# ooowedyn/InkLayer

Hardware: AMD Instinct MI355X
Metric: sketches/sec end-to-end (GroundingDINO+SAM) at 1024x1024 (higher is better)
Workload: dtype f16 (MFMA, f32 accumulate; f32 residual/norm/softmax; split-f16 = fp32-grade operands for patch-embed, neck, mask decoder); 1 GPU; full GroundingDINO Swin-T + SAM ViT-H pipeline, batch=8 per GPU, 1024x1024 synthetic sketches, 16 boxes/sketch, random-init weights; global_batch=8, parallelism=image-parallel x1

## Files before the change

### include/inklayer_hip.h

```cpp
#ifndef INKLAYER_HIP_H
#define INKLAYER_HIP_H

#include <stdint.h>

#ifdef __cplusplus
extern "C" {
#endif

#define INK_ABI_VERSION 8
int ink_abi_version(void);

typedef struct InkGemm {
  const void* A;
  const void* W;
  const float* bias;
  const float* col_scale;
  const float* residual;
  const int32_t* row_map;
  void* C;
  int32_t M, N, K;
  int32_t lda, ldw, ldr, ldc;
  int32_t act;
  int32_t c_f16;
} InkGemm;
// ... 119 lines not shown
                     int64_t ldo, void* stream);

int ink_attn_fewq(const void* Q, int64_t ldq, const void* K, int64_t ldk, const void* V, int64_t ldv,
                  int32_t n_batch, int32_t n_q, int32_t n_k, int32_t n_heads, int32_t head_dim, float scale,
                  const int32_t* q_batch_rows, const int32_t* kv_batch_rows, const float* k_add, void* O, int64_t ldo,
                  void* stream);

int ink_biattn_colstats(const float* scores, int32_t B, int32_t S, int32_t HT, float* part_ws, float* stats, void* stream);

int ink_fusion_fold_workspace(int32_t B, int32_t S, int64_t* out_floats);
int ink_fusion_fold(float* v_f32, int32_t B, int32_t S, const float* lnv_g, const float* lnv_b, float eps,
                    const float* text_k_f32, const float* text_vl_f32, int64_t ld_text, int32_t T, const void* Wq_f16,
                    const float* bq, const void* Wvv_f16, const float* bvv, const void* Wo_f16, const float* bo,
                    const float* gamma_v, float scale, float* ws, void* out_l_f16, const float* pos, void* out16_pos,
                    void* out16, void* stream);

int ink_sam_upscale_pack(const void* ws_f16, void* blob_f16, void* stream);
int ink_sam_upscale_tail(const float* u0, int64_t ld_tok, int32_t n, int32_t g, const float* ln_g, const float* ln_b, float eps,
                         const void* blob_f16, const float* b3, const float* hyper, int32_t n_masks, float* low,
                         void* stream);

int ink_proj256_ln_pack(const void* ws_f16, void* blob_f16, void* stream);
int ink_proj256_ln(const float* a_f32, const void* blob_f16, const float* bias, const float* res_f32,
                   const int32_t* res_batch_rows, int32_t rows_per_batch, const float* ln_g, const float* ln_b, float eps,
                   int64_t rows, float* out_f32, void* out_split_f16, void* stream);

int ink_ffn256_pack_bytes(int32_t hid, int32_t with_pre, int64_t* out_bytes);
int ink_ffn256_pack(const void* w1_f16, const float* b1, const void* w2_f16, int32_t hid, const void* wpre_f16, void* blob,
                    void* stream);
int ink_ffn256_fused(const void* x_f16, int64_t ldx, const float* res_f32, const void* blob, const float* b2,
                     const float* ln_g, const float* ln_b, float eps, int32_t M, int32_t hid, const float* pre_bias,
                     const float* pre_ln_g, const float* pre_ln_b, float* out_f32, void* stream);

int ink_topk_rowmax(const float* logits, int32_t B, int32_t S, int32_t T, int32_t K, int32_t* out_idx,
                    float* out_val, void* cand_ws, void* stream);

int ink_sine_embed4(const float* ref, const float* dim_t, int32_t N, void* out_f16, void* stream);

int ink_box_refine(const float* delta, int64_t ldd, const float* ref, int32_t N, int32_t ref_is_logit,
                   float* out, void* stream);

int ink_mask_cleanup_workspace_ints(int32_t n, int32_t H, int32_t W, int32_t k, int64_t* out_ints);
int ink_mask_cleanup(const void* masks_u8, int32_t n, int32_t H, int32_t W, int32_t k, int32_t area_threshold,
                     double aspect_threshold, void* tmp_a_u8, void* tmp_b_u8, int32_t* workspace, void* out_u8,
                     void* stream);

int ink_mask_sketch_iou_counts(const void* masks_u8, const void* sketch_rgb_u8, int32_t n, int32_t H, int32_t W,
                               void* bits_ws_u64, int32_t* counts, void* stream);

int ink_sam_amg_stats(const float* low, int32_t n, const int32_t* index, int32_t m, const int32_t* m_dev, int32_t S,
                      int32_t L, int32_t in_h, int32_t in_w, int32_t crop_h, int32_t crop_w, double thr, double offset,
                      int32_t x0, int32_t y0, int32_t orig_h, int32_t orig_w, int32_t* table, void* planes_u64,
                      float* out_logits, void* stream);

int ink_mask_rle_counts(const void* planes_u64, const int32_t* select, int32_t k, int32_t H, int32_t W,
                        int32_t* n_counts, void* stream);
int ink_mask_rle_write(const void* planes_u64, const int32_t* select, int32_t k, int32_t H, int32_t W,
                       const int32_t* offsets, int32_t* counts, void* stream);

int ink_mask_small_regions_workspace_ints(int32_t k, int32_t H, int32_t W, int64_t* out_ints);
int ink_mask_small_regions(const void* planes_u64, int32_t k, int32_t H, int32_t W, int32_t min_area, int32_t holes,
                           void* tmp_planes_u64, int32_t* workspace, void* out_planes_u64, int32_t* changed, void* stream);

int ink_box_nms(const float* boxes, const float* scores, int32_t n, float iou_threshold, void* workspace_u64,
                int32_t* keep, int32_t* n_keep, void* stream);

// ... 114 lines not shown
```

### inklayer_amd/_lib.py

```python
from __future__ import annotations

import ctypes as C
import os
from pathlib import Path

_LIB_PATH = Path(__file__).resolve().parent / "lib" / "libinklayer_hip.so"
_lib = None

c_void_p, c_int, c_i64, c_float = C.c_void_p, C.c_int32, C.c_int64, C.c_float


class InkGemm(C.Structure):
    _fields_ = [
        ("A", c_void_p), ("W", c_void_p), ("bias", c_void_p), ("col_scale", c_void_p),
        ("residual", c_void_p), ("row_map", c_void_p), ("C", c_void_p),
        ("M", c_int), ("N", c_int), ("K", c_int),
        ("lda", c_int), ("ldw", c_int), ("ldr", c_int), ("ldc", c_int),
        ("act", c_int), ("c_f16", c_int),
    ]


class InkAttn(C.Structure):
    _fields_ = [
        ("Q", c_void_p), ("K", c_void_p), ("V", c_void_p), ("O", c_void_p),
# ... 40 lines not shown
                               c_void_p],
    "ink_box_nms": [c_void_p, c_void_p, c_int, c_float, c_void_p, c_void_p, c_void_p, c_void_p],
    "ink_ms_deform_attn_forward": [c_void_p, C.POINTER(c_i64), C.POINTER(c_i64), c_void_p, c_void_p, c_int,
                                   c_int, c_int, c_int, c_int, c_int, c_int, c_int, c_void_p, c_void_p],
    "ink_ms_deform_attn_forward_dev": [c_void_p, c_void_p, c_void_p, c_void_p, c_void_p, c_int, c_int, c_int, c_int,
                                       c_int, c_int, c_int, c_int, c_int, c_void_p, c_void_p],
    "ink_ms_deform_attn_backward_dev": [c_void_p, c_void_p, c_void_p, c_void_p, c_void_p, c_void_p, c_int, c_int, c_int,
                                        c_int, c_int, c_int, c_int, c_int, c_int, c_void_p, c_void_p, c_void_p,
                                        c_void_p],
    "ink_msda_fused": [c_void_p, c_void_p, c_i64, c_void_p, c_int, c_i64, c_i64, C.POINTER(c_int), c_int,
                       c_int, c_int, c_void_p, c_void_p],
    "ink_swin_patchify": [c_void_p, c_int, c_int, C.POINTER(c_float), C.POINTER(c_float), c_void_p, c_void_p],
    "ink_layernorm_merge4": [c_void_p, c_i64, c_void_p, c_void_p, c_float, c_void_p, c_int, c_int, c_void_p,
                             c_void_p],
    "ink_groupnorm_nhwc": [c_void_p, c_int, c_int, c_int, c_int, c_void_p, c_void_p, c_float, c_void_p,
                           c_void_p, c_i64, c_void_p],
    "ink_gather_rows": [c_void_p, c_i64, c_i64, c_void_p, c_i64, c_int, c_int, c_int, c_void_p, c_void_p,
                        c_void_p],
    "ink_biattn_fusion": [c_void_p, c_void_p, c_int, c_int, c_int, c_int, c_float, c_void_p, c_void_p,
                          c_void_p, c_int, c_void_p, c_void_p, c_void_p],
    "ink_biattn_colstats": [c_void_p, c_int, c_int, c_int, c_void_p, c_void_p, c_void_p],
    "ink_fusion_fold_workspace": [c_int, c_int, C.POINTER(c_i64)],
    "ink_relpos_bias64_f16": [c_void_p, c_i64, c_void_p, c_void_p, c_int, c_int, c_int, c_float, c_void_p, c_void_p, c_void_p],
    "ink_proj256_ln_pack": [c_void_p, c_void_p, c_void_p],
    "ink_proj256_ln": [c_void_p, c_void_p, c_void_p, c_void_p, c_void_p, c_int, c_void_p, c_void_p, c_float, c_i64, c_void_p,
                       c_void_p, c_void_p],
    "ink_sam_upscale_pack": [c_void_p, c_void_p, c_void_p],
    "ink_sam_upscale_tail": [c_void_p, c_i64, c_int, c_int, c_void_p, c_void_p, c_float, c_void_p, c_void_p, c_void_p,
                             c_int, c_void_p, c_void_p],
    "ink_ffn256_pack_bytes": [c_int, c_int, C.POINTER(c_i64)],
    "ink_ffn256_pack": [c_void_p, c_void_p, c_void_p, c_int, c_void_p, c_void_p, c_void_p],
    "ink_ffn256_fused": [c_void_p, c_i64, c_void_p, c_void_p, c_void_p, c_void_p, c_void_p, c_float, c_int, c_int,
                         c_void_p, c_void_p, c_void_p, c_void_p, c_void_p],
    "ink_fusion_fold": [c_void_p, c_int, c_int, c_void_p, c_void_p, c_float, c_void_p, c_void_p, c_i64, c_int, c_void_p,
                        c_void_p, c_void_p, c_void_p, c_void_p, c_void_p, c_void_p, c_float, c_void_p, c_void_p, c_void_p,
                        c_void_p, c_void_p, c_void_p],
    "ink_attn_fewkeys": [c_void_p, c_i64, c_void_p, c_i64, c_void_p, c_i64, c_int, c_int, c_int, c_int, c_int,
                         c_float, c_void_p, c_void_p, c_void_p, c_int, c_void_p, c_i64, c_void_p],
    "ink_attn_fewq": [c_void_p, c_i64, c_void_p, c_i64, c_void_p, c_i64, c_int, c_int, c_int, c_int, c_int,
                      c_float, c_void_p, c_void_p, c_void_p, c_void_p, c_i64, c_void_p],
    "ink_topk_rowmax": [c_void_p, c_int, c_int, c_int, c_int, c_void_p, c_void_p, c_void_p, c_void_p],
    "ink_sine_embed4": [c_void_p, c_void_p, c_int, c_void_p, c_void_p],
    "ink_box_refine": [c_void_p, c_i64, c_void_p, c_int, c_int, c_void_p, c_void_p],
    "ink_mask_cleanup_workspace_ints": [c_int, c_int, c_int, c_int, C.POINTER(c_i64)],
    "ink_mask_cleanup": [c_void_p, c_int, c_int, c_int, c_int, c_int, C.c_double, c_void_p, c_void_p, c_void_p,
                         c_void_p, c_void_p],
    "ink_mask_sketch_iou_counts": [c_void_p, c_void_p, c_int, c_int, c_int, c_void_p, c_void_p, c_void_p],
    "ink_refine_sketch_planes": [c_void_p, c_int, c_int, c_void_p, c_void_p, c_void_p],
    "ink_bitplane_pack": [c_void_p, c_int, c_int, c_int, c_int, c_void_p, c_void_p],
    "ink_refine_depth_samples": [c_void_p, c_int, c_void_p, c_void_p, c_int, c_int, c_int, c_void_p, c_void_p, c_void_p],
    "ink_refine_pair_tables": [c_void_p, c_void_p, c_int, c_int, c_int, c_void_p, c_void_p, c_void_p, c_void_p,
                               c_void_p, c_void_p],
    "ink_refine_composite": [c_void_p, c_void_p, c_int, c_int, c_int, c_void_p, c_void_p, c_void_p],
    "ink_refine_relabel_clean": [c_void_p, c_void_p, c_int, c_int, c_void_p, c_void_p],
    "ink_refine_grow_workspace": [c_int, c_int, C.POINTER(c_i64), C.POINTER(c_i64)],
    "ink_refine_grow": [c_void_p, c_void_p, c_int, c_int, c_void_p, c_void_p, c_void_p, c_void_p, c_void_p, c_void_p,
                        c_int, c_void_p, c_void_p],
    "ink_refine_query_dists": [c_void_p, c_void_p, c_void_p, c_int, c_int, c_int, c_void_p, c_void_p],
    "ink_refine_finalize": [c_void_p, c_void_p, c_int, c_void_p, c_int, c_int, c_void_p, c_void_p, c_void_p, c_void_p],
    "ink_host_sparse_sample": [c_void_p, c_int, c_int, c_void_p, c_int, c_void_p],
    "ink_host_assign_unlabeled": [c_void_p, c_int, c_void_p, c_int, c_void_p, c_void_p, c_void_p, c_int, c_void_p],
    "ink_depth_patchify": [c_void_p, c_int, c_int, c_int, c_int, c_int, c_int, C.POINTER(C.c_double), C.POINTER(C.c_double),
                           c_int, c_void_p, c_void_p],
    "ink_resize_bilinear_ac_nhwc": [c_void_p, c_int, c_int, c_int, c_int, c_int, c_int, c_void_p, c_void_p, c_void_p],
    "ink_im2col3x3_ex_f16": [c_void_p, c_int, c_int, c_int, c_int, c_int, c_int, c_void_p, c_void_p],
    "ink_layers_otsu_planes": [c_void_p, c_int, c_int, c_int, c_int, c_void_p, c_void_p, c_void_p, c_void_p],
# ... 64 lines not shown
```

### inklayer_amd/build.py

```python
from __future__ import annotations

import os
import subprocess
import sys
from concurrent.futures import ThreadPoolExecutor
from pathlib import Path

ROOT = Path(__file__).resolve().parent
CSRC = ROOT / "csrc"
LIBDIR = ROOT / "lib"
OBJDIR = LIBDIR / "obj"
LIB = LIBDIR / "libinklayer_hip.so"
HIPCC = os.environ.get("HIPCC", "/opt/rocm/bin/hipcc")
FLAGS = ["--offload-arch=gfx950", "-O3", "-std=c++17", "-fPIC", "-ffp-contract=off",
         "-mllvm", "-amdgpu-mfma-vgpr-form",

         "-Wall", "-Wno-unused-function", "-Wno-unused-variable"]


def _newest_header() -> float:
    hs = list(CSRC.glob("*.h")) + list((ROOT.parent / "include").glob("*.h"))
    return max(h.stat().st_mtime for h in hs)


NO_SPILL = {"ffn_fused.hip", "proj_ln.hip", "amg.hip", "layers.hip", "inpaint_ops.hip", "visualize.hip"}


def _check_no_spill(src: Path, remarks: str) -> None:
    name = None
    for line in remarks.splitlines():
        if "Function Name:" in line:
            name = line.split("Function Name:")[1].split("[")[0].strip()
        elif "ScratchSize [bytes/lane]:" in line:
            n = int(line.split("ScratchSize [bytes/lane]:")[1].split("[")[0])
            if n != 0:
                raise RuntimeError(f"{src.name}: kernel {name} spills ({n} bytes of scratch per lane) - the kernels of "
                                   f"this file must stay in registers (see NO_SPILL); reduce register pressure")


def _compile(src: Path, force: bool, hdr_time: float) -> Path:
    obj = OBJDIR / (src.stem + ".o")
    if (not force and obj.exists() and obj.stat().st_mtime > src.stat().st_mtime
            and obj.stat().st_mtime > hdr_time):
        return obj
    guard = src.name in NO_SPILL
    cmd = [HIPCC, *FLAGS, *(["-Rpass-analysis=kernel-resource-usage", "-fno-caret-diagnostics"] if guard else []), "-c", str(src), "-o", str(obj)]
    r = subprocess.run(cmd, capture_output=True, text=True)
    if r.returncode != 0:
        raise RuntimeError(f"hipcc failed for {src.name}:\n{r.stdout}\n{r.stderr}")
    err = r.stderr
    if guard:
        try:
            _check_no_spill(src, err)
        except RuntimeError:
            obj.unlink(missing_ok=True)
            raise
        err = "\n".join(l for l in err.splitlines()
                        if "kernel-resource-usage" not in l and not l.startswith("In file included from"))
# ... 28 lines not shown
```

### inklayer_amd/gdino.py

```python
from __future__ import annotations

import math
from dataclasses import dataclass
from typing import Dict, List, Optional, Sequence, Tuple

import numpy as np
import torch

from . import ops
from ._lru import LRU

F16, F32, I32 = torch.float16, torch.float32, torch.int32


@dataclass
class GDinoConfig:
    embed_dim: int = 96
    depths: Tuple[int, ...] = (2, 2, 6, 2)
    num_heads: Tuple[int, ...] = (3, 6, 12, 24)
    window_size: int = 7
    out_indices: Tuple[int, ...] = (1, 2, 3)
    hidden_dim: int = 256
    nheads: int = 8
    enc_layers: int = 6
# ... 137 lines not shown
            refs.append(torch.stack((rx.reshape(-1) / ww, ry.reshape(-1) / hh), -1))
            gy, gx = torch.meshgrid(torch.linspace(0, hh - 1, hh), torch.linspace(0, ww - 1, ww), indexing="ij")
            grid = (torch.stack((gx, gy), -1) + 0.5) / torch.tensor([float(ww), float(hh)])
            props.append(torch.cat((grid, torch.ones_like(grid) * 0.05 * (2.0 ** lvl)), -1).view(-1, 4))
        self.enc_ref = torch.cat(refs, 0).to(dev).contiguous()
        pr = torch.cat(props, 0)
        valid = ((pr > 0.01) & (pr < 0.99)).all(-1)
        pr = torch.log(pr / (1 - pr)).masked_fill(~valid[:, None], float("inf"))
        self.props_unsig = pr.to(dev).contiguous()
        self.valid_map = torch.where(valid, torch.arange(self.S), torch.full((self.S,), -1)).to(I32).to(dev)


def swin_dense_bias(table: torch.Tensor, ws: int, nh: int, scale: float) -> torch.Tensor:
    co = torch.stack(torch.meshgrid(torch.arange(ws), torch.arange(ws), indexing="ij")).flatten(1)
    rel = (co[:, :, None] - co[:, None, :]).permute(1, 2, 0).contiguous()
    rel[:, :, 0] += ws - 1
    rel[:, :, 1] += ws - 1
    rel[:, :, 0] *= 2 * ws - 1
    rel_index = rel.sum(-1).view(-1)
    bias = torch.zeros((nh, ws * ws, 64))
    bias[:, :, :ws * ws] = table[rel_index].view(ws * ws, ws * ws, nh).permute(2, 0, 1) / scale
    return bias


def clean_state_dict(sd: Dict[str, torch.Tensor]) -> Dict[str, torch.Tensor]:
    if any(k.startswith("module.") for k in sd):
        return {(k[7:] if k.startswith("module.") else k): v for k, v in sd.items()}
    return sd


class GDinoEngine:
    fuse_ffn = True
    fuse_ffn_pre = True
    fold_fusion = True

    def __init__(self, state_dict: Dict[str, torch.Tensor], cfg: Optional[GDinoConfig] = None,
                 device: str | torch.device = "cuda", encoded_text: Optional[torch.Tensor] = None,
                 token_ids: Sequence[int] = DEFAULT_TOKEN_IDS):
        cfg = cfg or GDinoConfig()
        self.cfg, self.dev = cfg, torch.device(device)
        assert self.dev.type == "cuda", "the InkLayer detector runs on MI355X only"
        assert cfg.hidden_dim == 256 and cfg.nheads == 8 and cfg.num_feature_levels == 4 and cfg.n_points == 4
        assert all(cfg.embed_dim * 2 ** i // nh == 32 for i, nh in enumerate(cfg.num_heads))
        sd, dev = clean_state_dict(state_dict), self.dev
        self.w: Dict[str, torch.Tensor] = {}
        w = self.w

        def h(name, shape=None):
            t = sd[name].detach().to(torch.float32)
            return (t.reshape(shape) if shape is not None else t).to(dev, F16).contiguous()

        def f(name):
            return ops.own_f32(sd[name], dev)

        def lin(dst, src):
            w[dst + ".w"], w[dst + ".b"] = h(src + ".weight"), f(src + ".bias")

        def ln(dst, src):
            w[dst + ".w"], w[dst + ".b"] = f(src + ".weight"), f(src + ".bias")

        def cat_lin(dst, srcs):
            w[dst + ".w"] = torch.cat([h(s + ".weight") for s in srcs]).contiguous()
            w[dst + ".b"] = torch.cat([f(s + ".bias") for s in srcs]).contiguous()

        bb = "backbone.0."
        pw = sd[bb + "patch_embed.proj.weight"].detach().to(torch.float32).cpu().reshape(cfg.embed_dim, 48)
        w["pe.w"] = torch.cat([pw, torch.zeros(cfg.embed_dim, 16)], 1).to(dev, F16).contiguous()
        w["pe.b"] = f(bb + "patch_embed.proj.bias")
        ln("pe.norm", bb + "patch_embed.norm")
        ws = cfg.window_size
        scale = 32 ** -0.5
        for i, (dep, nh) in enumerate(zip(cfg.depths, cfg.num_heads)):
            for b in range(dep):
                p, d = f"{bb}layers.{i}.blocks.{b}.", f"s{i}b{b}"
                ln(d + ".norm1", p + "norm1")
                ln(d + ".norm2", p + "norm2")
                lin(d + ".qkv", p + "attn.qkv")
                lin(d + ".proj", p + "attn.proj")
                lin(d + ".fc1", p + "mlp.fc1")
                lin(d + ".fc2", p + "mlp.fc2")
                tab = sd[p + "attn.relative_position_bias_table"].detach().to(torch.float32).cpu()
                w[d + ".bias"] = swin_dense_bias(tab, ws, nh, scale).to(dev).contiguous()
            if i < len(cfg.depths) - 1:
                ln(f"s{i}.merge.norm", f"{bb}layers.{i}.downsample.norm")
                w[f"s{i}.merge.w"] = h(f"{bb}layers.{i}.downsample.reduction.weight")
            if i in cfg.out_indices:
                ln(f"s{i}.outnorm", f"{bb}norm{i}")
        for l in range(cfg.num_feature_levels):
            cw = sd[f"input_proj.{l}.0.weight"].detach().to(torch.float32)
            if cw.shape[-1] == 1:
                w[f"ip{l}.w"] = cw.reshape(cw.shape[0], cw.shape[1]).to(dev, F16).contiguous()
            else:
                w[f"ip{l}.w"] = cw.permute(0, 2, 3, 1).reshape(cw.shape[0], -1).to(dev, F16).contiguous()
            w[f"ip{l}.b"] = f(f"input_proj.{l}.0.bias")
            ln(f"ip{l}.gn", f"input_proj.{l}.1")
        t = "transformer."
        self.level_embed_cpu = sd[t + "level_embed"].detach().to(torch.float32).cpu()

        def msda(dst, src):
            cat_lin(dst + ".proj", [src + "sampling_offsets", src + "attention_weights"])
            lin(dst + ".value", src + "value_proj")
            lin(dst + ".out", src + "output_proj")

        def mha(dst, src):
            W, b = sd[src + "in_proj_weight"].detach().to(torch.float32), sd[src + "in_proj_bias"].detach().to(torch.float32)
            D = W.shape[1]
            w[dst + ".qk.w"], w[dst + ".qk.b"] = W[:2 * D].to(dev, F16).contiguous(), b[:2 * D].to(dev).contiguous()
            w[dst + ".q.w"], w[dst + ".q.b"] = W[:D].to(dev, F16).contiguous(), b[:D].to(dev).contiguous()
            w[dst + ".kv.w"], w[dst + ".kv.b"] = W[D:].to(dev, F16).contiguous(), b[D:].to(dev).contiguous()
            w[dst + ".v.w"], w[dst + ".v.b"] = W[2 * D:].to(dev, F16).contiguous(), b[2 * D:].to(dev).contiguous()
            lin(dst + ".out", src + "out_proj")

        for i in range(cfg.enc_layers):
            p, d = f"{t}encoder.layers.{i}.", f"e{i}"
            msda(d + ".msda", p + "self_attn.")
# ... 75 lines not shown
            torch.cuda.current_stream(self.dev).wait_stream(side)
            graph = torch.cuda.CUDAGraph()
            with torch.cuda.graph(graph):
                out = self._forward_eager(static_in)
            g = (graph, static_in, out, self.plan(h, w_, B))
            self._graphs.put(key, g)
        graph, static_in, out = g[:3]
        for dst, src in zip(static_in, images_u8):
            dst.copy_(src)
        graph.replay()
        return out[0].clone(), out[1].clone()

    def plan(self, h: int, w: int, B: int) -> _Plan:
        return self._plans.get_or_make((h, w, B), lambda: _Plan(self, h, w, B))

    def _mlp3(self, prefix: str, x16: torch.Tensor) -> torch.Tensor:
        w = self.w
        a = ops.gemm(x16, w[prefix + "0.w"], w[prefix + "0.b"], act="relu", out_dtype=F16)
        a = ops.gemm(a, w[prefix + "1.w"], w[prefix + "1.b"], act="relu", out_dtype=F16)
        return ops.gemm(a, w[prefix + "2.w"], w[prefix + "2.b"])

    def _swin_block(self, x: torch.Tensor, i: int, b: int, pl: _Plan) -> None:
        cfg, w = self.cfg, self.w
        C, nh, nW = cfg.embed_dim * 2 ** i, cfg.num_heads[i], pl.nW[i]
        d = f"s{i}b{b}"
        shifted = b % 2 == 1
        wm = pl.win_map[i][1 if shifted else 0]
        y = ops.layernorm_rows(x, w[d + ".norm1.w"], w[d + ".norm1.b"], 1e-5, gather=wm)
        qkv = ops.gemm(y, w[d + ".qkv.w"], w[d + ".qkv.b"], out_dtype=F16)
        o = ops.flash_attn(qkv[:, :C], qkv[:, C:2 * C], qkv[:, 2 * C:], n_batch=pl.B * nW, n_heads=nh,
                           head_dim=32, scale=32 ** -0.5, n_q=49, n_k=49, dense_bias=w[d + ".bias"],
                           dense_mask=pl.shift_mask[i] if shifted else None)
        ops.gemm(o, w[d + ".proj.w"], w[d + ".proj.b"], residual=x, row_map=wm, out=x)
        y = ops.layernorm_rows(x, w[d + ".norm2.w"], w[d + ".norm2.b"], 1e-5)
        hmid = ops.gemm(y, w[d + ".fc1.w"], w[d + ".fc1.b"], act="gelu", out_dtype=F16)
        ops.gemm(hmid, w[d + ".fc2.w"], w[d + ".fc2.b"], residual=x, out=x)

    def backbone(self, images_u8: Sequence[torch.Tensor], pl: _Plan) -> Dict[int, Tuple[torch.Tensor, torch.Tensor]]:
        cfg, w, dev = self.cfg, self.w, self.dev
        B = len(images_u8)
        H0, W0 = pl.stage_hw[0]
        T0 = H0 * W0
        patches = torch.empty((B * T0, 64), device=dev, dtype=F16)
        for b, img in enumerate(images_u8):
            ops.swin_patchify(img, cfg.pixel_mean, cfg.pixel_std, patches[b * T0:(b + 1) * T0])
        x = ops.gemm(patches, w["pe.w"], w["pe.b"])
        x = ops.layernorm_rows(x, w["pe.norm.w"], w["pe.norm.b"], 1e-5, out_dtype=F32)
        outs = {}
        for i, dep in enumerate(cfg.depths):
            for b in range(dep):
                self._swin_block(x, i, b, pl)
            if i in cfg.out_indices:
                o32 = torch.empty_like(x)
                o16 = torch.empty(x.shape, device=dev, dtype=F16)
                ops.layernorm_rows(x, w[f"s{i}.outnorm.w"], w[f"s{i}.outnorm.b"], 1e-5, out=o32, out2=o16)
                outs[i] = (o32, o16)
            if i < len(cfg.depths) - 1:
                m = ops.layernorm_merge4(x, w[f"s{i}.merge.norm.w"], w[f"s{i}.merge.norm.b"], 1e-5, pl.merge_map[i])
                x = ops.gemm(m, w[f"s{i}.merge.w"])
        return outs

    def neck(self, feats, pl: _Plan, B: int) -> torch.Tensor:
        cfg, w, dev = self.cfg, self.w, self.dev
        S = pl.S
        src = torch.empty((B * S, 256), device=dev, dtype=F32)
        nfeat = len(cfg.out_indices)
# ... 201 lines not shown
```

### inklayer_amd/ops.py

```python
from __future__ import annotations

import ctypes as C
from typing import Optional, Sequence, Tuple

import torch

from . import _lib
from ._lib import InkAttn, InkGemm, check

ACT = {None: 0, "none": 0, "gelu": 1, "relu": 2}
F16, F32 = torch.float16, torch.float32


_GEMM_TRACE = None


def set_gemm_trace(lst) -> None:
    global _GEMM_TRACE
    _GEMM_TRACE = lst


_ATTN_TRACE = None


# ... 770 lines not shown
    assert tuple(w1.shape) == (hid, 256) and tuple(w2.shape) == (256, hid)
    assert b1.dtype == F32 and b1.is_contiguous() and b1.numel() == hid
    assert w_pre is None or (w_pre.dtype == F16 and w_pre.is_contiguous() and tuple(w_pre.shape) == (256, 256))
    need = C.c_int64(0)
    check(_lib.lib().ink_ffn256_pack_bytes(hid, int(w_pre is not None), C.byref(need)), "ink_ffn256_pack_bytes")
    blob = torch.empty(need.value // 2, device=w1.device, dtype=F16)
    check(_lib.lib().ink_ffn256_pack(w1.data_ptr(), b1.data_ptr(), w2.data_ptr(), hid, _p(w_pre), blob.data_ptr(), _stream()),
          "ink_ffn256_pack")
    return blob


def ffn256_fused(x16: torch.Tensor, res: torch.Tensor, blob: torch.Tensor, hid: int, b2: torch.Tensor,
                 ln_g: torch.Tensor, ln_b: torch.Tensor, eps: float, out: Optional[torch.Tensor] = None,
                 pre: Optional[Tuple[torch.Tensor, torch.Tensor, torch.Tensor]] = None) -> torch.Tensor:
    M = int(x16.shape[0])
    assert x16.dtype == F16 and x16.stride(1) == 1 and x16.shape[1] == 256
    assert res.dtype == F32 and res.is_contiguous() and tuple(res.shape) == (M, 256)
    need = C.c_int64(0)
    check(_lib.lib().ink_ffn256_pack_bytes(hid, int(pre is not None), C.byref(need)), "ink_ffn256_pack_bytes")
    assert blob.dtype == F16 and blob.numel() * 2 == need.value and b2.dtype == F32
    assert b2.numel() == 256 and ln_g.numel() == 256 and ln_b.numel() == 256 and ln_g.dtype == F32 and ln_b.dtype == F32
    if pre is not None:
        assert all(t.dtype == F32 and t.is_contiguous() and t.numel() == 256 for t in pre)
    if out is None:
        out = torch.empty_like(res)
    assert out.dtype == F32 and out.is_contiguous() and tuple(out.shape) == (M, 256)
    pb, pg, pe = pre if pre is not None else (None, None, None)
    check(_lib.lib().ink_ffn256_fused(x16.data_ptr(), x16.stride(0), res.data_ptr(), blob.data_ptr(), b2.data_ptr(),
                                      ln_g.data_ptr(), ln_b.data_ptr(), eps, M, hid, _p(pb), _p(pg), _p(pe), out.data_ptr(),
                                      _stream()), "ink_ffn256_fused")
    return out


def attn_fewkeys(q: torch.Tensor, k: torch.Tensor, v: torch.Tensor, *, B: int, n_heads: int, head_dim: int,
                 scale: float, blocked: Optional[torch.Tensor] = None, n_q: Optional[int] = None,
                 q_batch_rows: Optional[torch.Tensor] = None, q_add: Optional[torch.Tensor] = None) -> torch.Tensor:
    io = q.dtype
    for t in (q, k, v):
        assert t.dtype == io and io in (F16, F32) and t.dim() == 2 and t.stride(1) == 1
        assert t.data_ptr() % 16 == 0
    if n_q is None:
        n_q = q.shape[0] // B
    n_k = k.shape[0] // B
    out = torch.empty((B * n_q, n_heads * head_dim), device=q.device, dtype=io)
    if blocked is not None:
        assert blocked.dtype == torch.uint8 and blocked.is_contiguous() and blocked.shape == (n_q, n_k)
    if q_batch_rows is not None:
        assert q_batch_rows.dtype == torch.int32 and q_batch_rows.numel() == B and q_batch_rows.is_cuda
    if q_add is not None:
        assert q_add.dtype == F32 and q_add.is_contiguous() and tuple(q_add.shape) == (n_q, n_heads * head_dim)
    check(_lib.lib().ink_attn_fewkeys(q.data_ptr(), q.stride(0), k.data_ptr(), k.stride(0), v.data_ptr(),
                                      v.stride(0), B, n_q, n_k, n_heads, head_dim, scale, _p(blocked),
                                      _p(q_batch_rows), _p(q_add), int(io == F32), out.data_ptr(), out.stride(0), _stream()),
          "ink_attn_fewkeys")
    return out


def attn_fewq(q: torch.Tensor, k: torch.Tensor, v: torch.Tensor, *, n_batch: int, n_heads: int, head_dim: int,
              scale: float, n_q: int, n_k: int, q_batch_rows: Optional[torch.Tensor] = None,
              kv_batch_rows: Optional[torch.Tensor] = None, k_add: Optional[torch.Tensor] = None) -> torch.Tensor:
    for t in (q, k, v):
        assert t.dtype == F32 and t.dim() == 2 and t.stride(1) == 1
        assert t.data_ptr() % 16 == 0
    for rows in (q_batch_rows, kv_batch_rows):
        assert rows is None or (rows.dtype == torch.int32 and rows.numel() == n_batch and rows.is_cuda)
    out = torch.empty((n_batch * n_q, n_heads * head_dim), device=q.device, dtype=F32)
# ... 393 lines not shown
```

Measured before the change: 118.4 sketches/s.

## Fuse Swin stage-0/1 MLP (LN, fc1, GELU, fc2, residual) into one kernel

Adds a fused HIP kernel for the Swin-T MLP block at C=96 and C=192. It applies layernorm in registers, streams pre-packed fc1/fc2 weight chunks through double-buffered LDS, and accumulates fc2 output on top of the residual, so the hidden activation never touches global memory. The fc1 bias is folded into an extra K slice as a split f16 pair. This removes three kernel launches and the f16 hidden-tensor round trip per block. The costs are a custom weight layout, f16 rounding of the LN output, and a tight register/LDS budget.

```diff
diff --git a/include/inklayer_hip.h b/include/inklayer_hip.h
--- a/include/inklayer_hip.h
+++ b/include/inklayer_hip.h
@@ -175,6 +175,12 @@
                      const float* ln_g, const float* ln_b, float eps, int32_t M, int32_t hid, const float* pre_bias,
                      const float* pre_ln_g, const float* pre_ln_b, float* out_f32, void* stream);
 
+int ink_swin_mlp_pack_bytes(int32_t C, int64_t* out_bytes);
+int ink_swin_mlp_pack(const void* w1_f16, const float* b1, const void* w2_f16, int32_t C, int32_t hid, void* blob,
+                      void* stream);
+int ink_swin_mlp_fused(float* x_f32, const void* blob, const float* ln_g, const float* ln_b, const float* b2, float eps,
+                       int32_t M, int32_t C, int32_t hid, void* stream);
+
 int ink_topk_rowmax(const float* logits, int32_t B, int32_t S, int32_t T, int32_t K, int32_t* out_idx,
                     float* out_val, void* cand_ws, void* stream);
 
diff --git a/inklayer_amd/_lib.py b/inklayer_amd/_lib.py
--- a/inklayer_amd/_lib.py
+++ b/inklayer_amd/_lib.py
@@ -96,6 +96,9 @@
     "ink_ffn256_pack": [c_void_p, c_void_p, c_void_p, c_int, c_void_p, c_void_p, c_void_p],
     "ink_ffn256_fused": [c_void_p, c_i64, c_void_p, c_void_p, c_void_p, c_void_p, c_void_p, c_float, c_int, c_int,
                          c_void_p, c_void_p, c_void_p, c_void_p, c_void_p],
+    "ink_swin_mlp_pack_bytes": [c_int, C.POINTER(c_i64)],
+    "ink_swin_mlp_pack": [c_void_p, c_void_p, c_void_p, c_int, c_int, c_void_p, c_void_p],
+    "ink_swin_mlp_fused": [c_void_p, c_void_p, c_void_p, c_void_p, c_void_p, c_float, c_int, c_int, c_int, c_void_p],
     "ink_fusion_fold": [c_void_p, c_int, c_int, c_void_p, c_void_p, c_float, c_void_p, c_void_p, c_i64, c_int, c_void_p,
                         c_void_p, c_void_p, c_void_p, c_void_p, c_void_p, c_void_p, c_float, c_void_p, c_void_p, c_void_p,
                         c_void_p, c_void_p, c_void_p],
diff --git a/inklayer_amd/build.py b/inklayer_amd/build.py
--- a/inklayer_amd/build.py
+++ b/inklayer_amd/build.py
@@ -23,7 +23,7 @@
     return max(h.stat().st_mtime for h in hs)
 
 
-NO_SPILL = {"ffn_fused.hip", "proj_ln.hip", "amg.hip", "layers.hip", "inpaint_ops.hip", "visualize.hip"}
+NO_SPILL = {"ffn_fused.hip", "swin_fused.hip", "proj_ln.hip", "amg.hip", "layers.hip", "inpaint_ops.hip", "visualize.hip"}
 
 
 def _check_no_spill(src: Path, remarks: str) -> None:
diff --git a/inklayer_amd/csrc/swin_fused.hip b/inklayer_amd/csrc/swin_fused.hip
--- /dev/null
+++ b/inklayer_amd/csrc/swin_fused.hip
@@ -0,0 +1,271 @@
+#include <type_traits>
+#include "common.h"
+#include "../../include/inklayer_hip.h"
+
+namespace {
+
+typedef __attribute__((address_space(1))) const void* gptr_t;
+typedef __attribute__((address_space(3))) void* lptr_t;
+typedef __attribute__((address_space(3))) char* lds_char_ptr;
+
+constexpr int BM = 128;
+constexpr int BLK = 1024;
+
+template <int C> struct Geo {
+  static_assert(C == 96 || C == 192, "Swin-T stages 0 and 1");
+  static constexpr int HC = C == 96 ? 64 : 32;
+  static constexpr int DEPTH = 6;
+  static constexpr int KA = C / 16 + 1;
+  static constexpr int JT = HC / 32;
+  static constexpr int KB = HC / 16;
+  static constexpr int NT = C / 32;
+  static constexpr int W1_BLKS = JT * KA;
+  static constexpr int W2_BLKS = NT * KB;
+  static constexpr int NBLK = W1_BLKS + W2_BLKS;
+  static constexpr int CHUNK = NBLK * BLK;
+  static constexpr int LDS_BYTES = 2 * CHUNK;
+  static constexpr int NSLOT = (NBLK + 3) / 4;
+  static_assert(2 * NSLOT <= NBLK, "the chunk loop issues every piece");
+  static constexpr int NPASS = C == 96 ? 1 : 2;
+  static constexpr int CW = C / NPASS;
+  static constexpr int OROW = CW * 4 + 16;
+  static_assert(4 * 32 * OROW <= 2 * CHUNK, "epilogue staging fits the (then free) weight buffers");
+  static_assert(LDS_BYTES <= 160 * 1024, "LDS budget");
+  static_assert((32 * CW / 4) % 64 == 0, "whole store instructions");
+};
+
+template <int I> using ic = std::integral_constant<int, I>;
+template <int I, int N, class F>
+__device__ __forceinline__ void static_for(F&& f) {
+  if constexpr (I < N) {
+    f(ic<I>{});
+    static_for<I + 1, N>(f);
+  }
+}
+template <int OFF>
+__device__ __forceinline__ f16x8 lds_frag(uint32_t addr) {
+  f16x8 v;
+  asm volatile("ds_read_b128 %0, %1 offset:%2" : "=v"(v) : "v"(addr), "n"(OFF));
+  return v;
+}
+template <int N>
+__device__ __forceinline__ void wait_frag(f16x8& f) {
+  asm volatile("s_waitcnt lgkmcnt(%1)" : "+v"(f) : "n"(N));
+}
+__device__ __forceinline__ f32x16 mfma32(const f16x8& a, const f16x8& b, const f32x16& c) {
+  return __builtin_amdgcn_mfma_f32_32x32x16_f16(a, b, c, 0, 0, 0);
+}
+
+__host__ __device__ constexpr int hid_perm(int p) { return (p & 7) < 4 ? 4 * (p >> 3) + (p & 7) : 8 + 4 * (p >> 3) + (p & 7) - 4; }
+
+__global__ __launch_bounds__(256) void swin_mlp_pack_kernel(const f16* __restrict__ W1, const float* __restrict__ b1,
+                                                            const f16* __restrict__ W2, int C, int HC,
+                                                            f16* __restrict__ blob) {
+  const int HID = 4 * C, KA = C / 16 + 1, KB = HC / 16, W1_BLKS = (HC / 32) * KA, NBLK = W1_BLKS + (C / 32) * KB;
+  const int64_t idx = (int64_t)blockIdx.x * 256 + threadIdx.x;
+  if (idx >= (int64_t)(HID / HC) * NBLK * 64) return;
+  const int lane = (int)(idx & 63);
+  const int q = (int)((idx >> 6) % NBLK);
+  const int c = (int)((idx >> 6) / NBLK);
+  const int l = lane & 31, hh = lane >> 5;
+  f16x8 v = {0, 0, 0, 0, 0, 0, 0, 0};
+  if (q < W1_BLKS) {
+    const int jt = q / KA, s = q % KA;
+    const int j = c * HC + 32 * jt + l;
+    if (s < C / 16) {
+      const f16* src = W1 + (int64_t)j * C + 16 * s;
+#pragma unroll
+      for (int e = 0; e < 8; ++e) v[e] = src[hid_perm(8 * hh + e)];
+    } else if (hh == 0) {
+      const f16 hi = (f16)b1[j];
+      v[0] = hi;
+      v[1] = (f16)(b1[j] - (float)hi);
+    }
+  } else {
+    const int nt = (q - W1_BLKS) / KB, s = (q - W1_BLKS) % KB;
+    const f16* src = W2 + (int64_t)(32 * nt + l) * HID + c * HC + 16 * s;
+#pragma unroll
+    for (int e = 0; e < 8; ++e) v[e] = src[hid_perm(8 * hh + e)];
+  }
+  *(f16x8*)(blob + idx * 8) = v;
+}
+
+template <int C>
+__device__ __forceinline__ void swin_mlp_body(float* __restrict__ x, const f16* __restrict__ blob,
+                                              const float* __restrict__ ln_g, const float* __restrict__ ln_b,
+                                              const float* __restrict__ b2, float eps, int M, char* smem) {
+  using G = Geo<C>;
+  constexpr int KA = G::KA, JT = G::JT, KB = G::KB, NT = G::NT, W1_BLKS = G::W1_BLKS, NBLK = G::NBLK, CHUNK = G::CHUNK;
+  constexpr int nchunk = 4 * C / G::HC, DEPTH = G::DEPTH;
+  const int tid = threadIdx.x, lane = tid & 63;
+  const int wave = __builtin_amdgcn_readfirstlane(tid >> 6);
+  const int l = lane & 31, hh = lane >> 5;
+  const int ntiles = (M + BM - 1) / BM;
+  const int m0 = xcd_remap(blockIdx.x, ntiles) * BM + wave * 32;
+  const int row = min(m0 + l, M - 1);
+
+  auto stage = [&](int buf, int c, int k) {
+    const int q = min(4 * k + wave, NBLK - 1);
+    __builtin_amdgcn_global_load_lds((gptr_t)((const char*)blob + (int64_t)c * CHUNK + q * BLK + lane * 16),
+                                     (lptr_t)(smem + buf * CHUNK + q * BLK), 16, 0, 0);
+  };
+#pragma unroll
+  for (int k = 0; k < G::NSLOT; ++k) stage(0, 0, k);
+
+  f32x16 y[NT];
+  const float* rp = x + (int64_t)row * C + 4 * hh;
+#pragma unroll
+  for (int nt = 0; nt < NT; ++nt)
+#pragma unroll
+    for (int g = 0; g < 4; ++g) {
+      const f32x4 r4 = *(const f32x4*)(rp + 32 * nt + 8 * g);
+#pragma unroll
+      for (int e = 0; e < 4; ++e) y[nt][4 * g + e] = r4[e];
+    }
+  float sum = 0.f;
+#pragma unroll
+  for (int nt = 0; nt < NT; ++nt)
+#pragma unroll
+    for (int r = 0; r < 16; ++r) sum += y[nt][r];
+  sum += __shfl_xor(sum, 32, 64);
+  const float mean = sum * (1.0f / C);
+  float sq = 0.f;
+#pragma unroll
+  for (int nt = 0; nt < NT; ++nt)
+#pragma unroll
+    for (int r = 0; r < 16; ++r) {
+      const float d = y[nt][r] - mean;
+      sq += d * d;
+    }
+  sq += __shfl_xor(sq, 32, 64);
+  const float rstd = 1.0f / sqrtf(sq * (1.0f / C) + eps);
+  f16x8 xf[KA];
+#pragma unroll
+  for (int nt = 0; nt < NT; ++nt)
+#pragma unroll
+    for (int g = 0; g < 4; ++g) {
+      const int col = 32 * nt + 8 * g;
+      const f32x4 g0 = *(const f32x4*)(ln_g + col), g1 = *(const f32x4*)(ln_g + col + 4);
+      const f32x4 e0 = *(const f32x4*)(ln_b + col), e1 = *(const f32x4*)(ln_b + col + 4);
+      const f32x4 c0 = *(const f32x4*)(b2 + col), c1 = *(const f32x4*)(b2 + col + 4);
+#pragma unroll
+      for (int e = 0; e < 4; ++e) {
+        const float v = y[nt][4 * g + e];
+        xf[2 * nt + (g >> 1)][4 * (g & 1) + e] = (f16)((v - mean) * rstd * (hh ? g1[e] : g0[e]) + (hh ? e1[e] : e0[e]));
+        y[nt][4 * g + e] = v + (hh ? c1[e] : c0[e]);
+      }
+    }
+  xf[C / 16] = (f16x8){0, 0, 0, 0, 0, 0, 0, 0};
+  if (hh == 0) xf[C / 16][0] = xf[C / 16][1] = (f16)1.0f;
+
+  const uint32_t lds0 = (uint32_t)(uintptr_t)(lds_char_ptr)smem + lane * 16;
+  const f32x16 zero = {0.f, 0.f, 0.f, 0.f, 0.f, 0.f, 0.f, 0.f, 0.f, 0.f, 0.f, 0.f, 0.f, 0.f, 0.f, 0.f};
+  for (int c = 0; c < nchunk; ++c) {
+    asm volatile("s_waitcnt vmcnt(0)" ::: "memory");
+    __builtin_amdgcn_s_barrier();
+    asm volatile("" ::: "memory");
+    const int cn = min(c + 1, nchunk - 1);
+    const uint32_t wa = lds0 + (c & 1) * CHUNK;
+    const uint32_t wb = wa + W1_BLKS * BLK;
+    f16x8 fr[DEPTH + 1];
+
+    auto read = [&](auto ii) {
+      constexpr int i = decltype(ii)::value;
+      if constexpr (i < W1_BLKS) fr[i % (DEPTH + 1)] = lds_frag<((i % JT) * KA + i / JT) * BLK>(wa);
+      else fr[i % (DEPTH + 1)] = lds_frag<(((i - W1_BLKS) % NT) * KB + (i - W1_BLKS) / NT) * BLK>(wb);
+    };
+    static_for<0, DEPTH>(read);
+    f32x16 h[JT];
+    f16x8 hf;
+    static_for<0, NBLK>([&](auto ii) {
+      constexpr int i = decltype(ii)::value;
+      if constexpr (i + DEPTH < NBLK) read(ic<i + DEPTH>{});
+      wait_frag<(NBLK - 1 - i < DEPTH ? NBLK - 1 - i : DEPTH)>(fr[i % (DEPTH + 1)]);
+      if constexpr (i < W1_BLKS) {
+        constexpr int s = i / JT, jt = i % JT;
+        h[jt] = mfma32(fr[i % (DEPTH + 1)], xf[s], s == 0 ? zero : h[jt]);
+      } else {
+        constexpr int s = (i - W1_BLKS) / NT, nt = (i - W1_BLKS) % NT;
+        if constexpr (nt == 0) {
+#pragma unroll
+          for (int e = 0; e < 8; ++e) hf[e] = (f16)gelu_erf(h[s >> 1][8 * (s & 1) + e]);
+        }
+        y[nt] = mfma32(fr[i % (DEPTH + 1)], hf, y[nt]);
+      }
+      if constexpr (i % 2 == 1 && i / 2 < G::NSLOT) stage((c + 1) & 1, cn, i / 2);
+    });
+  }
+
+  asm volatile("s_waitcnt vmcnt(0)" ::: "memory");
+  __syncthreads();
+  char* ot = smem + wave * 32 * G::OROW;
+  constexpr int PIECES = G::CW / 4;
+#pragma unroll
+  for (int ps = 0; ps < G::NPASS; ++ps) {
+#pragma unroll
+    for (int t = 0; t < NT / G::NPASS; ++t)
+#pragma unroll
+      for (int g = 0; g < 4; ++g) {
+        f32x4 v;
+#pragma unroll
+        for (int e = 0; e < 4; ++e) v[e] = y[ps * (NT / G::NPASS) + t][4 * g + e];
+        *(f32x4*)(ot + l * G::OROW + (32 * t + 8 * g + 4 * hh) * 4) = v;
+      }
+#pragma unroll 4
+    for (int it = 0; it < 32 * PIECES / 64; ++it) {
+      const int idx = it * 64 + lane, r = idx / PIECES, pc = idx % PIECES;
+      const f32x4 v = *(const f32x4*)(ot + r * G::OROW + pc * 16);
+      if (m0 + r < M) *(f32x4*)(x + (int64_t)(m0 + r) * C + ps * G::CW + pc * 4) = v;
+    }
+  }
+}
+
+template <int C>
+__global__ __launch_bounds__(256) __attribute__((amdgpu_waves_per_eu(2, 2))) void swin_mlp_kernel(
+    float* __restrict__ x, const f16* __restrict__ blob, const float* __restrict__ ln_g, const float* __restrict__ ln_b,
+    const float* __restrict__ b2, float eps, int M) {
+  extern __shared__ __attribute__((aligned(16))) char smem[];
+  swin_mlp_body<C>(x, blob, ln_g, ln_b, b2, eps, M, smem);
+}
+
+bool swin_c_ok(int C) { return C == 96 || C == 192; }
+int64_t swin_blob_bytes(int C) {
+  return C == 96 ? (int64_t)(4 * 96 / Geo<96>::HC) * Geo<96>::CHUNK : (int64_t)(4 * 192 / Geo<192>::HC) * Geo<192>::CHUNK;
+}
+
+}
+
+extern "C" int ink_swin_mlp_pack_bytes(int32_t C, int64_t* out_bytes) {
+  INK_CHECK_ARG(out_bytes && swin_c_ok(C));
+  *out_bytes = swin_blob_bytes(C);
+  return INK_OK;
+}
+
+extern "C" int ink_swin_mlp_pack(const void* w1_f16, const float* b1, const void* w2_f16, int32_t C, int32_t hid, void* blob,
+                                 void* stream) {
+  INK_CHECK_ARG(w1_f16 && b1 && w2_f16 && blob && swin_c_ok(C) && hid == 4 * C);
+  INK_CHECK_ARG((((uintptr_t)w1_f16 | (uintptr_t)w2_f16 | (uintptr_t)blob) & 15) == 0 && ((uintptr_t)b1 & 3) == 0);
+  const int HC = C == 96 ? Geo<96>::HC : Geo<192>::HC;
+  const int64_t pieces = swin_blob_bytes(C) / 16;
+  hipLaunchKernelGGL(swin_mlp_pack_kernel, dim3((unsigned)((pieces + 255) / 256)), dim3(256), 0, (hipStream_t)stream,
+                     (const f16*)w1_f16, b1, (const f16*)w2_f16, C, HC, (f16*)blob);
+  return ink_launch_status();
+}
+
+extern "C" int ink_swin_mlp_fused(float* x_f32, const void* blob, const float* ln_g, const float* ln_b, const float* b2,
+                                  float eps, int32_t M, int32_t C, int32_t hid, void* stream) {
+  INK_CHECK_ARG(x_f32 && blob && ln_g && ln_b && b2 && M > 0 && swin_c_ok(C) && hid == 4 * C);
+  INK_CHECK_ARG((((uintptr_t)x_f32 | (uintptr_t)blob | (uintptr_t)ln_g | (uintptr_t)ln_b | (uintptr_t)b2) & 15) == 0);
+  static bool attr = ((void)hipFuncSetAttribute((const void*)swin_mlp_kernel<96>, hipFuncAttributeMaxDynamicSharedMemorySize,
+                                                Geo<96>::LDS_BYTES),
+                      (void)hipFuncSetAttribute((const void*)swin_mlp_kernel<192>, hipFuncAttributeMaxDynamicSharedMemorySize,
+                                                Geo<192>::LDS_BYTES), true);
+  (void)attr;
+  const dim3 grid((unsigned)((M + BM - 1) / BM)), block(256);
+  hipStream_t st = (hipStream_t)stream;
+  if (C == 96)
+    hipLaunchKernelGGL(swin_mlp_kernel<96>, grid, block, Geo<96>::LDS_BYTES, st, x_f32, (const f16*)blob, ln_g, ln_b, b2, eps, M);
+  else
+    hipLaunchKernelGGL(swin_mlp_kernel<192>, grid, block, Geo<192>::LDS_BYTES, st, x_f32, (const f16*)blob, ln_g, ln_b, b2, eps, M);
+  return ink_launch_status();
+}
diff --git a/inklayer_amd/gdino.py b/inklayer_amd/gdino.py
--- a/inklayer_amd/gdino.py
+++ b/inklayer_amd/gdino.py
@@ -193,6 +193,7 @@
 class GDinoEngine:
     fuse_ffn = True
     fuse_ffn_pre = True
+    fuse_swin = True
     fold_fusion = True
 
     def __init__(self, state_dict: Dict[str, torch.Tensor], cfg: Optional[GDinoConfig] = None,
@@ -242,6 +243,8 @@
                 lin(d + ".fc2", p + "mlp.fc2")
                 tab = sd[p + "attn.relative_position_bias_table"].detach().to(torch.float32).cpu()
                 w[d + ".bias"] = swin_dense_bias(tab, ws, nh, scale).to(dev).contiguous()
+                if w[d + ".fc1.w"].shape[1] in ops.SWIN_FUSED_C and w[d + ".fc1.w"].shape[0] == 4 * w[d + ".fc1.w"].shape[1]:
+                    w[d + ".mlp.blob"] = ops.swin_mlp_pack(w[d + ".fc1.w"], w[d + ".fc1.b"], w[d + ".fc2.w"])
             if i < len(cfg.depths) - 1:
                 ln(f"s{i}.merge.norm", f"{bb}layers.{i}.downsample.norm")
                 w[f"s{i}.merge.w"] = h(f"{bb}layers.{i}.downsample.reduction.weight")
@@ -383,6 +386,9 @@
                            head_dim=32, scale=32 ** -0.5, n_q=49, n_k=49, dense_bias=w[d + ".bias"],
                            dense_mask=pl.shift_mask[i] if shifted else None)
         ops.gemm(o, w[d + ".proj.w"], w[d + ".proj.b"], residual=x, row_map=wm, out=x)
+        if self.fuse_swin and (d + ".mlp.blob") in w:
+            ops.swin_mlp_fused(x, w[d + ".mlp.blob"], w[d + ".norm2.w"], w[d + ".norm2.b"], w[d + ".fc2.b"], 1e-5)
+            return
         y = ops.layernorm_rows(x, w[d + ".norm2.w"], w[d + ".norm2.b"], 1e-5)
         hmid = ops.gemm(y, w[d + ".fc1.w"], w[d + ".fc1.b"], act="gelu", out_dtype=F16)
         ops.gemm(hmid, w[d + ".fc2.w"], w[d + ".fc2.b"], residual=x, out=x)
diff --git a/inklayer_amd/ops.py b/inklayer_amd/ops.py
--- a/inklayer_amd/ops.py
+++ b/inklayer_amd/ops.py
@@ -826,6 +826,36 @@
     return out
 
 
+SWIN_FUSED_C = (96, 192)
+
+
+def swin_mlp_pack(w1: torch.Tensor, b1: torch.Tensor, w2: torch.Tensor) -> torch.Tensor:
+    hid, Cc = int(w1.shape[0]), int(w1.shape[1])
+    assert Cc in SWIN_FUSED_C and hid == 4 * Cc, (Cc, hid)
+    assert w1.dtype == F16 and w2.dtype == F16 and w1.is_contiguous() and w2.is_contiguous()
+    assert tuple(w2.shape) == (Cc, hid)
+    assert b1.dtype == F32 and b1.is_contiguous() and b1.numel() == hid
+    need = C.c_int64(0)
+    check(_lib.lib().ink_swin_mlp_pack_bytes(Cc, C.byref(need)), "ink_swin_mlp_pack_bytes")
+    blob = torch.empty(need.value // 2, device=w1.device, dtype=F16)
+    check(_lib.lib().ink_swin_mlp_pack(_p(w1), _p(b1), _p(w2), Cc, hid, _p(blob), _stream()), "ink_swin_mlp_pack")
+    return blob
+
+
+def swin_mlp_fused(x: torch.Tensor, blob: torch.Tensor, ln_g: torch.Tensor, ln_b: torch.Tensor, b2: torch.Tensor,
+                   eps: float) -> torch.Tensor:
+    M, Cc = int(x.shape[0]), int(x.shape[1])
+    assert Cc in SWIN_FUSED_C, Cc
+    assert x.dtype == F32 and x.is_contiguous() and x.dim() == 2 and M > 0
+    need = C.c_int64(0)
+    check(_lib.lib().ink_swin_mlp_pack_bytes(Cc, C.byref(need)), "ink_swin_mlp_pack_bytes")
+    assert blob.dtype == F16 and blob.numel() * 2 == need.value
+    assert all(t.dtype == F32 and t.is_contiguous() and t.numel() == Cc for t in (ln_g, ln_b, b2))
+    check(_lib.lib().ink_swin_mlp_fused(_p(x), _p(blob), _p(ln_g), _p(ln_b), _p(b2), eps, M, Cc, 4 * Cc, _stream()),
+          "ink_swin_mlp_fused")
+    return x
+
+
 def attn_fewkeys(q: torch.Tensor, k: torch.Tensor, v: torch.Tensor, *, B: int, n_heads: int, head_dim: int,
                  scale: float, blocked: Optional[torch.Tensor] = None, n_q: Optional[int] = None,
                  q_batch_rows: Optional[torch.Tensor] = None, q_add: Optional[torch.Tensor] = None) -> torch.Tensor:
```

New measurement: 119.3 sketches/s (median of 6 runs). About the same (+0.8%).
